# shopetan/mini-kube-scheduler

Hardware: AMD Instinct MI355X
Metric: pod-node evals/sec + pods placed/sec at 5k nodes, 1/2/4/8 MI355X (higher is better)
Workload: dtype u32 (bit-sliced: 32 pod-node pairs per lane-op); 1 GPU; C3 batched: 5000 nodes x 100000 pods per batch per GPU (pod-sharded over 1 GPU); the K batches through msh_schedule_batches_device, 32 per launch, one stream; nodes=5000, parallelism=pod-sharded x1, streams=1, submit=multi (32 batches per launch)

## Files before the change

include/minisched_hip.h:

```cpp
#ifndef MINISCHED_HIP_H
#define MINISCHED_HIP_H

#include <stddef.h>
#include <stdint.h>

#ifdef __cplusplus
extern "C" {
#endif

#define MSH_ABI_VERSION 8

typedef enum msh_err {
  MSH_OK = 0,
  MSH_ERR_INVALID = -1,
  MSH_ERR_NO_DEVICE = -2,
  MSH_ERR_HIP = -3,
  MSH_ERR_STATE = -4,
  MSH_ERR_UNSUPPORTED = -5,
  MSH_ERR_NOMEM = -6
} msh_err;

typedef enum msh_status {
  MSH_PLACED = 0,
  MSH_FIT_ERROR = 1,
  MSH_SCORE_ERROR = 2
} msh_status;

typedef enum msh_plugin_id {
  MSH_PLUGIN_NODE_UNSCHEDULABLE = 1,
  MSH_PLUGIN_NODE_NUMBER = 2,
  MSH_PLUGIN_SCORE_COLUMN0 = 16,
  MSH_PLUGIN_SCORE_COLUMN1 = 17,
  MSH_PLUGIN_SCORE_COLUMN2 = 18,
  MSH_PLUGIN_SCORE_COLUMN3 = 19
} msh_plugin_id;

typedef enum msh_normalize {
  MSH_NORMALIZE_NONE = 0,
  MSH_NORMALIZE_DEFAULT = 1,
  MSH_NORMALIZE_DEFAULT_REVERSE = 2,
  MSH_NORMALIZE_MINMAX = 3
} msh_normalize;

typedef struct msh_ctx msh_ctx;

int msh_abi_version(void);

int msh_device_count(int* out_count);

int msh_host_alloc(size_t bytes, void** out_ptr);
void msh_host_free(void* ptr);

int msh_create(int device, msh_ctx** out_ctx);
void msh_destroy(msh_ctx* ctx);

typedef struct msh_options {
  int32_t struct_size;
  int32_t batch_kernel;
  int32_t pair_planes;
  int32_t pair_noax;
  int32_t pair_slices;
  int32_t seq_waves;
  int32_t seq_split;
  int32_t seq_pod_waves;
  int32_t gen_keys;
  int32_t gen_nnkey;
} msh_options;
int msh_create_ex(int device, const msh_options* opts, msh_ctx** out_ctx);

const char* msh_last_error(const msh_ctx* ctx);

int msh_set_plugins(msh_ctx* ctx, const int32_t* filter_ids, int32_t nf,
                    const int32_t* score_ids, const int64_t* weights, int32_t ns);
int msh_set_plugins_ex(msh_ctx* ctx, const int32_t* filter_ids, int32_t nf,
                       const int32_t* prescore_ids, int32_t npre,
                       const int32_t* score_ids, const int64_t* weights,
                       const int32_t* normalize, int32_t ns);

typedef enum msh_tiebreak { MSH_TIEBREAK_FIRST = 0, MSH_TIEBREAK_RANDOM = 1 } msh_tiebreak;
int msh_set_tiebreak(msh_ctx* ctx, int32_t mode, uint64_t seed, uint64_t counter);
int msh_get_tiebreak(const msh_ctx* ctx, int32_t* out_mode, uint64_t* out_seed, uint64_t* out_counter);

int msh_upload_nodes(msh_ctx* ctx, int32_t n, const uint8_t* unsched, const int8_t* digit);
int msh_num_nodes(const msh_ctx* ctx, int32_t* out_n);

int msh_upload_score_column(msh_ctx* ctx, int32_t plugin_id, int32_t n, const int64_t* scores);

#define MSH_EXPORT_NONE ((int64_t)(-9223372036854775807LL - 1))
int msh_export_results(msh_ctx* ctx, int32_t p, const int8_t* pod_digit, const uint8_t* pod_tol,
                       uint8_t* out_filter, int64_t* out_score, int64_t* out_final);

int msh_patch_nodes(msh_ctx* ctx, int32_t count, const int32_t* idx, const uint8_t* unsched,
                    const int8_t* digit);

int msh_schedule_batch(msh_ctx* ctx, int32_t p, const int8_t* pod_digit, const uint8_t* pod_tol,
                       int32_t* out_idx, int64_t* out_score, int32_t* out_status);

#define MSH_ASYNC_DEPTH 4
int msh_schedule_batch_async(msh_ctx* ctx, int32_t p, const int8_t* pod_digit, const uint8_t* pod_tol,
                             int32_t* out_idx, int64_t* out_score, int32_t* out_status, uint64_t* out_ticket);
int msh_wait(msh_ctx* ctx, uint64_t ticket);

int msh_schedule_batch_device(msh_ctx* ctx, int32_t p, const int8_t* d_pod_digit,
                              const uint8_t* d_pod_tol, int32_t* d_out_idx,
                              int64_t* d_out_score, int32_t* d_out_status, void* stream);

#define MSH_BATCHES_PER_LAUNCH 32
typedef struct msh_batch {
  int32_t p;
  int32_t reserved;
  const int8_t* pod_digit;
  const uint8_t* pod_tol;
  int32_t* out_idx;
  int64_t* out_score;
  int32_t* out_status;
} msh_batch;
int msh_schedule_batches_device(msh_ctx* ctx, int32_t nb, const msh_batch* batches, void* stream);

typedef void (*msh_commit_cb)(void* user, int32_t pod, int32_t node_idx, int64_t score);
// ... 231 lines not shown
```

mini-kube-scheduler_amd/_native.py:

```python
from __future__ import annotations

import ctypes as C
import os
from pathlib import Path

import numpy as np

PKG_DIR = Path(__file__).resolve().parent
LIB_PATH = Path(os.environ.get("MSH_LIBRARY", PKG_DIR / "libminisched_hip.so"))

MSH_OK = 0
MSH_ERR_INVALID = -1
MSH_ERR_NO_DEVICE = -2
MSH_ERR_HIP = -3
MSH_ERR_STATE = -4
MSH_ERR_UNSUPPORTED = -5
MSH_ERR_NOMEM = -6
ERR_NAMES = {
    MSH_ERR_INVALID: "MSH_ERR_INVALID",
    MSH_ERR_NO_DEVICE: "MSH_ERR_NO_DEVICE",
    MSH_ERR_HIP: "MSH_ERR_HIP",
    MSH_ERR_STATE: "MSH_ERR_STATE",
    MSH_ERR_UNSUPPORTED: "MSH_ERR_UNSUPPORTED",
    MSH_ERR_NOMEM: "MSH_ERR_NOMEM",
# ... 45 lines not shown
    "msh_schedule_batches_device", "msh_schedule_sequential",
    "msh_schedule_sequential_device", "msh_node_pod_counts", "msh_reset_node_pod_counts",
    "msh_upload_node_capacity", "msh_patch_node_capacity", "msh_clear_node_capacity", "msh_node_capacity",
    "msh_upload_node_resources", "msh_patch_node_resources", "msh_clear_node_resources", "msh_node_resources",
    "msh_schedule_sequential_fit", "msh_schedule_sequential_fit_device",
    "msh_set_resource_score", "msh_get_resource_score", "msh_seq_fit_max_nodes",
    "msh_upload_node_zones", "msh_clear_node_zones", "msh_node_zones", "msh_set_spread_groups",
    "msh_get_spread_groups", "msh_spread_counts", "msh_patch_spread_counts", "msh_reset_spread_counts",
    "msh_seq_spread_max_nodes", "msh_schedule_sequential_spread", "msh_schedule_sequential_spread_device",
    "msh_seq_spread_scored_max_nodes", "msh_schedule_sequential_spread_scored",
    "msh_schedule_sequential_spread_scored_device",
    "msh_upload_node_class_bits", "msh_patch_node_class_bits", "msh_clear_node_class_bits", "msh_node_class_bits",
    "msh_seq_classes_max_nodes", "msh_schedule_sequential_classes", "msh_schedule_sequential_classes_device",
    "msh_upload_node_class_prefs", "msh_patch_node_class_prefs", "msh_clear_node_class_prefs", "msh_node_class_prefs",
    "msh_set_preference_weights", "msh_preference_weights", "msh_seq_prefs_max_nodes",
    "msh_schedule_sequential_prefs", "msh_schedule_sequential_prefs_device",
    "msh_set_spread_group_modes", "msh_get_spread_group_modes", "msh_set_spread_score_weight", "msh_spread_score_weight",
    "msh_spread_soft_weight", "msh_seq_soft_max_nodes", "msh_schedule_sequential_soft",
    "msh_schedule_sequential_soft_device",
    "msh_set_balanced_score", "msh_balanced_score", "msh_seq_balanced_max_nodes", "msh_schedule_sequential_balanced",
    "msh_schedule_sequential_balanced_device",
    "msh_set_pod_affinity_terms", "msh_get_pod_affinity_terms", "msh_set_pod_profiles", "msh_get_pod_profiles",
    "msh_upload_pod_affinity_state", "msh_patch_pod_affinity_state", "msh_pod_affinity_state",
    "msh_seq_podaffinity_max_nodes", "msh_schedule_sequential_podaffinity", "msh_schedule_sequential_podaffinity_device",
    "msh_shard_keys_len", "msh_shard_keys_device", "msh_decode_keys_device", "msh_keys_slot1_is_any",
    "msh_generic_ext_len", "msh_generic_extents_device", "msh_generic_best_device",
    "msh_generic_candidates_device", "msh_generic_decode_device",
    "msh_comm_unique_id", "msh_comm_init", "msh_comm_info", "msh_schedule_nodeshard_device", "msh_schedule_nodeshard",
    "msh_group_create", "msh_group_destroy", "msh_group_last_error", "msh_group_schedule_batch",
    "msh_timing_begin", "msh_timing_end",
    "msh_pack_nodes", "msh_pack_pods", "msh_toleration_tolerates_unschedulable",
)


class MshError(RuntimeError):
    def __init__(self, code: int, msg: str):
        super().__init__(f"{ERR_NAMES.get(code, code)}: {msg}")
        self.code = code


class Toleration(C.Structure):
    _fields_ = [("key", C.c_char_p), ("op", C.c_char_p), ("value", C.c_char_p), ("effect", C.c_char_p)]


class Batch(C.Structure):
    _fields_ = [("p", C.c_int32), ("reserved", C.c_int32), ("pod_digit", C.c_void_p), ("pod_tol", C.c_void_p),
                ("out_idx", C.c_void_p), ("out_score", C.c_void_p), ("out_status", C.c_void_p)]


class Options(C.Structure):
    _fields_ = [("struct_size", C.c_int32), ("batch_kernel", C.c_int32), ("pair_planes", C.c_int32),
                ("pair_noax", C.c_int32), ("pair_slices", C.c_int32), ("seq_waves", C.c_int32),
                ("seq_split", C.c_int32), ("seq_pod_waves", C.c_int32), ("gen_keys", C.c_int32),
                ("gen_nnkey", C.c_int32)]


OPTION_NAMES = {
    "batch_kernel": {"auto": 0, "pair": 0, "generic": 1},
    "pair_planes": {"auto": 0, "sgpr": 1, "lds": 2},
    "pair_noax": {"auto": 0, "noax": 1, "axlast": 2},
    "pair_slices": {"auto": 0},
    "seq_waves": {"auto": 0},
    "seq_split": {"auto": 0, "serial": 1, "blocks": 2},
    "seq_pod_waves": {"auto": 0},
    "gen_keys": {"auto": 0, "f53": 0, "u64": 1},
    "gen_nnkey": {"auto": 0, "select": 1},
}


def make_options(opts: dict | None) -> "Options | None":
    if not opts:
        return None
    o = Options()
    o.struct_size = C.sizeof(Options)
    for k, v in opts.items():
        if k not in OPTION_NAMES:
            raise ValueError(f"unknown msh_options field {k!r}")
        if isinstance(v, str):
            v = OPTION_NAMES[k][v] if v in OPTION_NAMES[k] else int(v)
        setattr(o, k, int(v))
    return o


COMM_ID_BYTES = 128
GROUP_MAX_SHARDS = 16
BATCHES_PER_LAUNCH = 32
ASYNC_DEPTH = 4

COMMIT_CB = C.CFUNCTYPE(None, C.c_void_p, C.c_int32, C.c_int32, C.c_int64)

_P = C.c_void_p
_I32 = C.c_int32
_I64 = C.c_int64

_SIGS = {
    "msh_abi_version": (C.c_int, []),
    "msh_device_count": (C.c_int, [C.POINTER(C.c_int)]),
    "msh_host_alloc": (C.c_int, [C.c_size_t, C.POINTER(_P)]),
    "msh_host_free": (None, [_P]),
    "msh_create": (C.c_int, [C.c_int, C.POINTER(_P)]),
    "msh_create_ex": (C.c_int, [C.c_int, C.POINTER(Options), C.POINTER(_P)]),
    "msh_destroy": (None, [_P]),
    "msh_last_error": (C.c_char_p, [_P]),
    "msh_set_tiebreak": (C.c_int, [_P, _I32, C.c_uint64, C.c_uint64]),
    "msh_get_tiebreak": (C.c_int, [_P, C.POINTER(_I32), C.POINTER(C.c_uint64), C.POINTER(C.c_uint64)]),
    "msh_set_plugins": (C.c_int, [_P, _P, _I32, _P, _P, _I32]),
    "msh_set_plugins_ex": (C.c_int, [_P, _P, _I32, _P, _I32, _P, _P, _P, _I32]),
    "msh_upload_nodes": (C.c_int, [_P, _I32, _P, _P]),
    "msh_num_nodes": (C.c_int, [_P, C.POINTER(_I32)]),
    "msh_upload_score_column": (C.c_int, [_P, _I32, _I32, _P]),
    "msh_patch_nodes": (C.c_int, [_P, _I32, _P, _P, _P]),
    "msh_export_results": (C.c_int, [_P, _I32, _P, _P, _P, _P, _P]),
    "msh_schedule_batch": (C.c_int, [_P, _I32, _P, _P, _P, _P, _P]),
    "msh_schedule_batch_device": (C.c_int, [_P, _I32, _P, _P, _P, _P, _P, _P]),
    "msh_schedule_batches_device": (C.c_int, [_P, _I32, _P, _P]),
    "msh_schedule_batch_async": (C.c_int, [_P, _I32, _P, _P, _P, _P, _P, C.POINTER(C.c_uint64)]),
    "msh_wait": (C.c_int, [_P, C.c_uint64]),
    "msh_timing_begin": (C.c_int, [_P, _I32]),
    "msh_timing_end": (C.c_int, [_P, C.POINTER(C.c_int32), C.POINTER(C.c_double), C.POINTER(C.c_double)]),
# ... 167 lines not shown
```

mini-kube-scheduler_amd/csrc/msh_capi.cpp:

```cpp
#include <hip/hip_runtime.h>

#include <algorithm>
#include <array>
#include <atomic>
#include <cmath>
#include <condition_variable>
#include <cstdio>
#include <cstdint>
#include <cstdlib>
#include <cstring>
#include <functional>
#include <initializer_list>
#include <iterator>
#include <mutex>
#include <new>
#include <optional>
#include <string>
#include <thread>
#include <vector>

#include "../../include/minisched_hip.h"
#include "msh_ctx.h"
#include "msh_internal.h"
#include "msh_pool.h"
// ... 569 lines not shown
    const CopyJob jobs[2] = {{c->h_stage + L.pd, pod_digit, (size_t)p}, {c->h_stage + L.pt, pod_tol, (size_t)p}};
    par_copy(jobs, 2);
    src_pd = reinterpret_cast<const int8_t*>(c->h_stage + L.pd);
    src_pt = c->h_stage + L.pt;
  }
  io.d_pd = static_cast<int8_t*>(pinned_device_ptr(src_pd));
  io.d_pt = static_cast<uint8_t*>(pinned_device_ptr(src_pt));
  if (!io.d_pd || !io.d_pt) return fail(c, MSH_ERR_HIP, "page-locked pod columns without a device address");
  if (io.staged) {
    io.h_idx = reinterpret_cast<int32_t*>(c->h_stage + L.idx);
    io.h_score = out_score ? reinterpret_cast<int64_t*>(c->h_stage + L.score) : nullptr;
    io.h_status = reinterpret_cast<int32_t*>(c->h_stage + L.status);
    io.o_idx = io.h_idx;
    io.o_score = io.h_score;
    io.o_status = io.h_status;
  } else {
    io.h_idx = out_idx;
    io.h_score = out_score;
    io.h_status = out_status;
    io.o_idx = static_cast<int32_t*>(di);
    io.o_score = static_cast<int64_t*>(ds);
    io.o_status = static_cast<int32_t*>(dt);
  }
  return MSH_OK;
}

int host_io_end(msh_ctx* c, int32_t p, int32_t* out_idx, int64_t* out_score, int32_t* out_status,
                const HostIO& io) {
  MSH_HIP(c, hipStreamSynchronize(c->stream));
  c->async_done = c->async_issued;
  if (io.staged) {
    const CopyJob jobs[3] = {{out_idx, io.h_idx, (size_t)p * sizeof(int32_t)},
                             {out_status, io.h_status, (size_t)p * sizeof(int32_t)},
                             {out_score, io.h_score, (size_t)p * sizeof(int64_t)}};
    par_copy(jobs, out_score ? 3 : 2);
  }
  return MSH_OK;
}

thread_local std::string g_create_err;

bool apply_options(const msh_options& o, msh::DeviceInfo& d, std::string* err) {
  auto in = [&](const char* name, int32_t v, std::initializer_list<int32_t> allowed) {
    for (int32_t a : allowed)
      if (v == a) return true;
    *err = std::string("msh_options.") + name + " = " + std::to_string(v) + ": not one of";
    for (int32_t a : allowed) *err += " " + std::to_string(a);
    return false;
  };
  if (!in("batch_kernel", o.batch_kernel, {0, 1}) || !in("pair_planes", o.pair_planes, {0, 1, 2}) ||
      !in("pair_noax", o.pair_noax, {0, 1, 2}) || !in("pair_slices", o.pair_slices, {0, 1, 2, 4}) ||
      !in("seq_waves", o.seq_waves, {0, 1, 4, 15, 16}) || !in("seq_split", o.seq_split, {0, 1, 2}) ||
      !in("seq_pod_waves", o.seq_pod_waves, {0, 1, 2, 4, 8}) ||
      !in("gen_keys", o.gen_keys, {0, 1}) || !in("gen_nnkey", o.gen_nnkey, {0, 1}))
    return false;
  d.batch_kernel = o.batch_kernel;
  d.pair_planes = o.pair_planes;
  d.pair_noax = o.pair_noax == 0 ? -1 : (o.pair_noax == 1 ? 1 : 0);
  d.bits_slices = o.pair_slices;
  d.seq_waves = o.seq_waves;
  d.seq_split = o.seq_split == 0 ? 2 : (o.seq_split == 1 ? 0 : 1);
  d.seq_pod_waves = o.seq_pod_waves;
  d.gen_f53 = o.gen_keys == 0 ? 1 : 0;
  d.gen_nnkey = o.gen_nnkey == 0 ? 1 : 0;
  return true;
}

}

using namespace msh::capi;

extern "C" {

int msh_abi_version(void) { return MSH_ABI_VERSION; }

int msh_device_count(int* out_count) {
  if (!out_count) return MSH_ERR_INVALID;
  int n = 0;
  hipError_t e = hipGetDeviceCount(&n);
  *out_count = (e == hipSuccess) ? n : 0;
  return MSH_OK;
}

int msh_host_alloc(size_t bytes, void** out_ptr) {
  if (!out_ptr) return MSH_ERR_INVALID;
  *out_ptr = nullptr;
  int n = 0;
  if (hipGetDeviceCount(&n) != hipSuccess || n <= 0) return MSH_ERR_NO_DEVICE;
  const size_t n_bytes = std::max<size_t>(bytes, 1);
  if (hipHostMalloc(out_ptr, n_bytes, hipHostMallocDefault) != hipSuccess) {
    *out_ptr = nullptr;
    return MSH_ERR_NOMEM;
  }
  const uintptr_t a = reinterpret_cast<uintptr_t>(*out_ptr);
  std::lock_guard<std::mutex> g(g_host_mu);
  g_host_allocs.insert(std::upper_bound(g_host_allocs.begin(), g_host_allocs.end(), std::make_pair(a, a)),
                       std::make_pair(a, a + n_bytes));
  return MSH_OK;
}

void msh_host_free(void* ptr) {
  if (!ptr) return;
  {
    const uintptr_t a = reinterpret_cast<uintptr_t>(ptr);
    std::lock_guard<std::mutex> g(g_host_mu);
    auto it = std::lower_bound(g_host_allocs.begin(), g_host_allocs.end(), std::make_pair(a, (uintptr_t)0));
    if (it != g_host_allocs.end() && it->first == a) g_host_allocs.erase(it);
  }
  (void)hipHostFree(ptr);
}

int msh_create(int device, msh_ctx** out_ctx) { return msh_create_ex(device, nullptr, out_ctx); }

int msh_create_ex(int device, const msh_options* opts, msh_ctx** out_ctx) {
  g_create_err.clear();
  if (!out_ctx) return MSH_ERR_INVALID;
  *out_ctx = nullptr;
// ... 1082 lines not shown
```

mini-kube-scheduler_amd/csrc/msh_internal.h:

```cpp
#pragma once

#include <hip/hip_runtime.h>

#include <cstdint>
#include <string>

namespace msh {

constexpr int32_t MAX_NODES = 0xFFFFFE;
constexpr int WAVE = 64;
constexpr int32_t GKEY_MAX = 0x7FFFFFFF;
constexpr uint32_t NOFIT = 0x80000000u;

struct PluginParams {
  int32_t has_nu_filter;
  int32_t has_nn_score;
  int32_t nn_prescore;
  int32_t mode;
  int64_t weight;
};

inline bool needs_kx(const PluginParams& pp) {
  return pp.has_nn_score && pp.nn_prescore && (pp.mode == 2 || pp.mode == 3);
}

struct DeviceInfo {
  int cus = 256;
  int bits_slices = 0;
  int seq_waves = 0;
  int batch_kernel = 0;
  int pair_planes = 0;
  int pair_noax = -1;
  int seq_split = 2;
  int seq_pod_waves = 0;
  int gen_f53 = 1;
  int gen_nnkey = 1;
};

constexpr uint32_t CODE_NONE_NODE = 15u;
constexpr uint32_t CODE_NONE_POD = 14u;

constexpr int PLANE_GW = 8;
constexpr int PLANE_N = 6;
constexpr int PLANE_X = 4, PLANE_V = 5;
constexpr int GROUP_NODES = PLANE_GW * 32;
constexpr int GROUP_DWORDS = PLANE_GW * PLANE_N;
constexpr int32_t NODE_PAD = 1024;

hipError_t launch_node_prep(const uint8_t* d_unsched, const int8_t* d_digit, int32_t n, int32_t n_pad,
                            int32_t has_nu, uint32_t* d_planes, hipStream_t s);
constexpr int PATCH_INLINE = 64;
struct TableCopyArgs {
  const uint8_t* src_unsched;
  const int8_t* src_digit;
  const uint32_t* src_planes;
  uint8_t* dst_unsched;
  int8_t* dst_digit;
  uint32_t* dst_planes;
  int32_t n, n_words, has_nu, count;
  unsigned long long inl[PATCH_INLINE];
};
hipError_t launch_table_copy(const TableCopyArgs& a, hipStream_t s);
hipError_t launch_patch_scatter(const unsigned long long* d_entries, int32_t count, uint8_t* d_unsched,
                                int8_t* d_digit, hipStream_t s);

constexpr int64_t EXPORT_NONE = INT64_MIN;
hipError_t launch_export(const uint8_t* d_unsched, const int8_t* d_digit, int32_t n,
                         const int8_t* d_pod_digit, const uint8_t* d_pod_tol, int32_t p,
                         const PluginParams& pp, uint8_t* d_filter, int64_t* d_raw, int64_t* d_fin,
                         hipStream_t s);

struct BatchDesc {
  const int8_t* pod_digit;
  const uint8_t* pod_tol;
  int32_t* out_idx;
  int64_t* out_score;
  int32_t* out_status;
  int32_t n_pods;
  int32_t reserved;
};
constexpr int MULTI_MAX = 32;

struct PairCommon {
  const uint32_t* planes;
  int32_t n_groups;
  int32_t g_full;
  int32_t gps;
  int32_t noax;
  int32_t nb;
  PluginParams pp;
  int64_t node_base;
  int32_t* keys;
  int32_t* counts;
  int64_t count_stride;
};
template <int NB>
struct PairArgsN : PairCommon {
  BatchDesc d[NB];
};
using PairArgs = PairArgsN<MULTI_MAX>;
hipError_t launch_pairs(PairArgs& a, bool shard, const DeviceInfo& dev, hipStream_t s);

struct PickArgs {
  const uint32_t* planes;
  int32_t n_groups;
  int32_t nb;
  PluginParams pp;
  uint64_t seed;
  BatchDesc d[MULTI_MAX];
  uint64_t draw_base[MULTI_MAX];
};
constexpr int TIEBREAK_LDS_MAX_GROUPS = 416;
hipError_t launch_pair_pick(const PickArgs& a, hipStream_t s);

hipError_t launch_decode_keys(const int8_t* pod_digit, int32_t p, const int32_t* keys, PluginParams pp,
                              int32_t* out_idx, int64_t* out_score, int32_t* out_status, hipStream_t s);

constexpr int GROUP_MAX = 16;
struct GroupPtrs {
  const int32_t* keys[GROUP_MAX];
  const int64_t* v[GROUP_MAX];
  const int32_t* idx[GROUP_MAX];
  int32_t n;
};
hipError_t launch_group_keys_decode(const GroupPtrs& g, const int8_t* pod_digit, int32_t p, PluginParams pp,
                                    int32_t* out_idx, int64_t* out_score, int32_t* out_status, hipStream_t s);
hipError_t launch_group_max_i64(const GroupPtrs& g, int64_t len, int64_t* out, hipStream_t s);
hipError_t launch_group_best_merge(const GroupPtrs& g, int32_t p, int64_t* out_total, int32_t* out_idx,
                                   hipStream_t s);

constexpr int GEN_MAX_SCORE = 5;
constexpr int GEN_COLS = 4;
struct GenericArgs {
// ... 171 lines not shown
```

mini-kube-scheduler_amd/csrc/msh_pair.hip:

```cpp
#include "msh_device.h"

namespace msh {

template <int NPL>
__device__ __forceinline__ void sload_group(u32x8* pl, const uint32_t* src) {
#pragma unroll
  for (int k = 0; k < NPL; ++k)
    asm volatile("s_load_dwordx8 %0, %1, %2" : "=s"(pl[k]) : "s"(src), "n"(k * PLANE_GW * 4));
  if constexpr (NPL == 5)
    asm volatile("s_waitcnt lgkmcnt(0)" : "+s"(pl[0]), "+s"(pl[1]), "+s"(pl[2]), "+s"(pl[3]), "+s"(pl[4]));
  else
    asm volatile("s_waitcnt lgkmcnt(0)" : "+s"(pl[0]), "+s"(pl[1]), "+s"(pl[2]), "+s"(pl[3]), "+s"(pl[4]),
                 "+s"(pl[5]));
}

__device__ __forceinline__ void sload_xv(u32x8 (&pl)[PLANE_N], const uint32_t* grp) {
  asm volatile("s_load_dwordx8 %0, %2, %3\n\ts_load_dwordx8 %1, %2, %4\n\ts_waitcnt lgkmcnt(0)"
               : "=&s"(pl[PLANE_X]), "=&s"(pl[PLANE_V])
               : "s"(grp), "n"(PLANE_X * PLANE_GW * 4), "n"(PLANE_V * PLANE_GW * 4));
}

template <int NPL, bool LDSP>
__device__ __forceinline__ void get_group(u32x8* pl, const uint32_t* planes, const uint4* s_tab, int32_t g) {
  if constexpr (LDSP) {
// ... 305 lines not shown
      uint32_t u = TY == 0 ? bop3_or_xor(pl[PLANE_X][ww], pl[0][ww], P0) : (pl[0][ww] ^ P0);
      u = bop3_or_xor(u, pl[1][ww], P1);
      u = bop3_or_xor(u, pl[2][ww], P2);
      t[h] = bop3_or_xor(u, pl[3][ww], P3);
    }
    am = bop3_and3(am, t[0], t[1]);
#pragma unroll
    for (int h = 0; h < 2; ++h) {
      const int ww = w + h;
      if constexpr (KX) {
        if constexpr (TY == 0) ax = PAD ? (ax | bop3_andn_and(t[h], pl[PLANE_X][ww], pl[PLANE_V][ww]))
                                       : bop3_or_andn(ax, t[h], pl[PLANE_X][ww]);
        else ax = PAD ? (ax | (t[h] & pl[PLANE_V][ww])) : (ax | t[h]);
      }
    }
  }
}

template <bool KX, int TY>
__device__ __forceinline__ void pair_group_hy(const uint32_t (&pl)[PLANE_N][PLANE_GW], const u32x8& X,
                                              const u32x8& D3, uint32_t P0, uint32_t P1, uint32_t P2, uint32_t P3,
                                              uint32_t nT, uint32_t& am, uint32_t& ax) {
#pragma unroll
  for (int w = 0; w < PLANE_GW; w += 2) {
    uint32_t t[2], xi[2];
#pragma unroll
    for (int h = 0; h < 2; ++h) {
      const int ww = w + h;
      uint32_t u;
      if constexpr (TY == 0) {
        u = bop3_or_xor(X[ww], pl[0][ww], P0);
      } else if constexpr (TY == 1) {
        u = pl[0][ww] ^ P0;
      } else {
        xi[h] = __builtin_amdgcn_bitop3_b32(X[ww], nT, nT, 0xc0);
        u = bop3_or_xor(xi[h], pl[0][ww], P0);
      }
      u = bop3_or_xor(u, pl[1][ww], P1);
      u = bop3_or_xor(u, pl[2][ww], P2);
      t[h] = bop3_or_xor(u, D3[ww], P3);
    }
    am = bop3_and3(am, t[0], t[1]);
    if constexpr (KX) {
#pragma unroll
      for (int h = 0; h < 2; ++h) {
        if constexpr (TY == 0) ax = bop3_or_andn(ax, t[h], X[w + h]);
        else if constexpr (TY == 1) ax |= t[h];
        else ax = bop3_or_andn(ax, t[h], xi[h]);
      }
    }
  }
}

template <int KIND>
__device__ __forceinline__ uint32_t group_first_lds(const uint4* __restrict__ s_tab, uint32_t g, uint32_t P0,
                                                    uint32_t P1, uint32_t P2, uint32_t P3, uint32_t nT) {
  const uint4* q = s_tab + g * (GROUP_DWORDS / 4);
#pragma unroll 1
  for (int hh = 0; hh < 2; ++hh) {
    uint32_t pl[PLANE_N][4];
#pragma unroll
    for (int k = 0; k < PLANE_N; ++k) {
      const uint4 v = q[2 * k + hh];
      pl[k][0] = v.x; pl[k][1] = v.y; pl[k][2] = v.z; pl[k][3] = v.w;
    }
    uint32_t t[4];
#pragma unroll
    for (int c = 0; c < 4; ++c) {
      const uint32_t fe = ~(pl[PLANE_X][c] & nT) & pl[PLANE_V][c];
      const uint32_t dm = (pl[0][c] ^ P0) | (pl[1][c] ^ P1) | (pl[2][c] ^ P2) | (pl[3][c] ^ P3);
      const uint32_t h = KIND == 1 ? (dm & fe) : (~dm & fe);
      t[c] = lowbit(h) | (uint32_t)(32 * c);
    }
    const uint32_t m = umin(umin(t[0], t[1]), umin(t[2], t[3]));
    if (m < 128u) return g * GROUP_NODES + (uint32_t)(hh * 128) + m;
  }
  return NOFIT;
}

template <bool KX>
__device__ __forceinline__ void group_firsts_lds(const uint4* __restrict__ s_tab, uint32_t g, uint32_t P0,
                                                 uint32_t P1, uint32_t P2, uint32_t P3, uint32_t nT, bool digit,
                                                 uint32_t& rm, uint32_t& rx) {
  const uint4* q = s_tab + g * (GROUP_DWORDS / 4);
  uint32_t bm = 0xFFFFFFFFu, bx = 0xFFFFFFFFu;
  if constexpr (!KX) {
    constexpr int PLX = 4;
    static_assert(PLANE_X == PLX, "X follows the four code planes");
    auto half = [&](auto hc) -> uint32_t {
      constexpr int hh = decltype(hc)::value;
      uint32_t pl[PLX + 1][4];
#pragma unroll
      for (int k = 0; k <= PLX; ++k) {
        const uint4 v = q[2 * k + hh];
        pl[k][0] = v.x; pl[k][1] = v.y; pl[k][2] = v.z; pl[k][3] = v.w;
      }
      uint32_t t[4];
#pragma unroll
      for (int c = 0; c < 4; ++c) {
        uint32_t u = __builtin_amdgcn_bitop3_b32(pl[PLX][c], nT, nT, 0xc0);
        u = bop3_or_xor(u, pl[0][c], P0);
        u = bop3_or_xor(u, pl[1][c], P1);
        u = bop3_or_xor(u, pl[2][c], P2);
        u = __builtin_amdgcn_bitop3_b32(u, pl[3][c], P3, 0x09);
        t[c] = lowbit(u);
        if (c + 4 * hh != 0) t[c] |= (uint32_t)(32 * (c + 4 * hh));
      }
      return umin(umin(t[0], t[1]), umin(t[2], t[3]));
    };
    bm = half(std::integral_constant<int, 0>{});
    if (__ballot(digit && bm == 0xFFFFFFFFu) != 0) bm = umin(bm, half(std::integral_constant<int, 1>{}));
    rm = bm < GROUP_NODES ? g * GROUP_NODES + bm : NOFIT;
    return;
  }
#pragma unroll 1
  for (int hh = 0; hh < 2; ++hh) {
    uint32_t pl[PLANE_N][4];
#pragma unroll
    for (int k = 0; k < PLANE_N; ++k) {
      const uint4 v = q[2 * k + hh];
      pl[k][0] = v.x; pl[k][1] = v.y; pl[k][2] = v.z; pl[k][3] = v.w;
    }
#pragma unroll
    for (int c = 0; c < 4; ++c) {
      const uint32_t fe = ~(pl[PLANE_X][c] & nT) & pl[PLANE_V][c];
      const uint32_t dm = (pl[0][c] ^ P0) | (pl[1][c] ^ P1) | (pl[2][c] ^ P2) | (pl[3][c] ^ P3);
      const uint32_t off = (uint32_t)(32 * (c + 4 * hh));
      bm = umin(bm, lowbit(~dm & fe) | off);
      if constexpr (KX) bx = umin(bx, lowbit(dm & fe) | off);
    }
    if (hh == 0 && __ballot((digit && bm == 0xFFFFFFFFu) || (KX && bx == 0xFFFFFFFFu)) == 0) break;
  }
  rm = bm < GROUP_NODES ? g * GROUP_NODES + bm : NOFIT;
  if constexpr (KX) rx = bx < GROUP_NODES ? g * GROUP_NODES + bx : NOFIT;
}

template <bool SHARD, bool KX, int W>
__global__ __launch_bounds__(W * WAVE) void pair_lds_kernel(PairArgs a) {
  constexpr bool CMP = KX && W == PL_WAVES;
  constexpr int HY = KX ? 2 : 1;
  extern __shared__ uint4 s_tab[];
  constexpr int NSL = W * PL_BPW;
  __shared__ uint32_t s_cnt[CMP ? NSL : 1];
  __shared__ uint32_t s_pod[CMP ? NSL * WAVE : 1];
  const BatchDesc& d = a.d[blockIdx.y];
  const int32_t np = d.n_pods;
  const int32_t wg0 = (int32_t)blockIdx.x * NSL * WAVE;
  if (wg0 >= np) return;
  {
    const uint4* __restrict__ src = reinterpret_cast<const uint4*>(a.planes);
    const int32_t nq = a.n_groups * (GROUP_DWORDS / 4);
    for (int32_t i = threadIdx.x; i < nq; i += W * WAVE) s_tab[i] = src[i];
  }
  const int lane = threadIdx.x & (WAVE - 1);
  const int wv = __builtin_amdgcn_readfirstlane((int)(threadIdx.x >> 6));
  const int32_t n_groups = a.n_groups, g_full = a.g_full;
  uint32_t pk[PL_BPW];
#pragma unroll
  for (int b = 0; b < PL_BPW; ++b) {
    const int32_t pos0 = (wv * PL_BPW + b) * WAVE + lane;
    const int32_t j = wg0 + pos0;
    uint32_t c = CODE_NONE_POD, t = 0u;
    if (j < np) {
      const int dq = d.pod_digit[j];
      c = (dq >= 0 && dq <= 9) ? (uint32_t)dq : CODE_NONE_POD;
      t = d.pod_tol[j] ? 1u : 0u;
    }
    pk[b] = ((uint32_t)pos0 << 8) | (t << 4) | c;
  }
  if constexpr (CMP) {
    uint64_t mn[PL_BPW];
#pragma unroll
    for (int b = 0; b < PL_BPW; ++b) {
      mn[b] = __ballot(((pk[b] >> 4) & 1u) == 0u);
      if (lane == 0) s_cnt[wv * PL_BPW + b] = (uint32_t)__builtin_popcountll(mn[b]);
    }
    __syncthreads();
    uint32_t tot = 0, pre[PL_BPW];
#pragma unroll
    for (int k = 0; k < NSL; ++k) {
      const uint32_t c = s_cnt[k];
#pragma unroll
      for (int b = 0; b < PL_BPW; ++b)
        if (k == wv * PL_BPW + b) pre[b] = tot;
      tot += c;
    }
#pragma unroll
    for (int b = 0; b < PL_BPW; ++b) {
      const uint32_t sl = (uint32_t)(wv * PL_BPW + b);
      const bool nt = ((pk[b] >> 4) & 1u) == 0u;
      const uint32_t below = nt ? __builtin_amdgcn_mbcnt_hi((uint32_t)(mn[b] >> 32), __builtin_amdgcn_mbcnt_lo((uint32_t)mn[b], 0u))
                                : __builtin_amdgcn_mbcnt_hi((uint32_t)(~mn[b] >> 32), __builtin_amdgcn_mbcnt_lo((uint32_t)~mn[b], 0u));
      const uint32_t pos = nt ? pre[b] + below : tot + (sl * WAVE - pre[b]) + below;
      s_pod[pos] = pk[b];
    }
    __syncthreads();
#pragma unroll
    for (int b = 0; b < PL_BPW; ++b) pk[b] = s_pod[(wv * PL_BPW + b) * WAVE + lane];
  } else {
    __syncthreads();
  }
  uint32_t P0[PL_BPW], P1[PL_BPW], P2[PL_BPW], P3[PL_BPW], nT[PL_BPW], code[PL_BPW];
  int32_t jj[PL_BPW];
  int ty[PL_BPW];
  bool any_act = false;
#pragma unroll
  for (int b = 0; b < PL_BPW; ++b) {
    const uint32_t c = pk[b] & 15u, t = (pk[b] >> 4) & 1u;
    jj[b] = wg0 + (int32_t)(pk[b] >> 8);
    code[b] = c;
    P0[b] = 0u - (c & 1u);
    P1[b] = 0u - ((c >> 1) & 1u);
    P2[b] = 0u - ((c >> 2) & 1u);
    P3[b] = 0u - (c >> 3);
    nT[b] = t ? 0u : 0xFFFFFFFFu;
    const uint64_t tm = __ballot(t != 0u);
    ty[b] = CMP ? (tm == 0 ? 0 : (~tm == 0 ? 1 : 2)) : 2;
    any_act = any_act || __ballot(jj[b] < np) != 0;
  }
  if (!any_act) return;
  uint32_t fm[PL_BPW], fx[PL_BPW], amw[PL_BPW];
#pragma unroll
  for (int b = 0; b < PL_BPW; ++b) {
    fm[b] = fx[b] = NO_GROUP;
    amw[b] = 0xFFFFFFFFu;
  }
  uint32_t fn = NO_GROUP, ft = NO_GROUP;
  uint32_t rm[PL_BPW], rx[PL_BPW];
  auto group0 = [&]() {
#pragma unroll
    for (int b = 0; b < PL_BPW; ++b) group_firsts_lds<KX>(s_tab, 0u, P0[b], P1[b], P2[b], P3[b], nT[b], code[b] != CODE_NONE_POD, rm[b], rx[b]);
  };
  auto scan = [&](auto noax) {
    constexpr bool NOAX = decltype(noax)::value;
    constexpr bool KXS = KX && !NOAX;
    for (int32_t g = n_groups - 1; g > 0; g -= 2) {
      uint32_t ams[PL_BPW], ax[PL_BPW];
      uint32_t(&am)[PL_BPW] = *(KX ? &ams : &amw);
#pragma unroll
      for (int b = 0; b < PL_BPW; ++b) {
        if constexpr (KX) am[b] = 0xFFFFFFFFu;
        ax[b] = 0u;
      }
      const int32_t g2 = g - 1 > 0 ? g - 1 : g;
      u32x8 spp[2][2];
      if constexpr (HY == 2) {
        asm volatile("s_load_dwordx8 %0, %4, %6\n\ts_load_dwordx8 %1, %4, %7\n\t"
                     "s_load_dwordx8 %2, %5, %6\n\ts_load_dwordx8 %3, %5, %7\n\ts_waitcnt lgkmcnt(0)"
                     : "=&s"(spp[0][0]), "=&s"(spp[0][1]), "=&s"(spp[1][0]), "=&s"(spp[1][1])
                     : "s"(a.planes + (size_t)g * GROUP_DWORDS), "s"(a.planes + (size_t)g2 * GROUP_DWORDS),
                       "n"(PLANE_X * PLANE_GW * 4), "n"(3 * PLANE_GW * 4));
      }
#pragma unroll
      for (int h = 0; h < 2; ++h) {
        const int32_t gg = h == 0 ? g : g - 1;
        if (h == 1 && gg <= 0) break;
        uint32_t pl[PLANE_N][PLANE_GW];
        if (!KX || gg < g_full) {
          u32x8 sp[2];
          if constexpr (HY == 2) {
            sp[0] = spp[h][0];
            sp[1] = spp[h][1];
          } else {
            asm volatile("s_load_dwordx8 %0, %2, %3\n\ts_load_dwordx8 %1, %2, %4\n\ts_waitcnt lgkmcnt(0)"
                         : "=&s"(sp[0]), "=&s"(sp[1])
                         : "s"(a.planes + (size_t)gg * GROUP_DWORDS), "n"(PLANE_X * PLANE_GW * 4), "n"(3 * PLANE_GW * 4));
          }
          lds_group<3>(pl, s_tab, gg);
#pragma unroll
          for (int b = 0; b < PL_BPW; ++b) {
            if (ty[b] == 0) pair_group_hy<KXS, 0>(pl, sp[0], sp[1], P0[b], P1[b], P2[b], P3[b], nT[b], am[b], ax[b]);
            else if (ty[b] == 1) pair_group_hy<KXS, 1>(pl, sp[0], sp[1], P0[b], P1[b], P2[b], P3[b], nT[b], am[b], ax[b]);
            else pair_group_hy<KXS, 2>(pl, sp[0], sp[1], P0[b], P1[b], P2[b], P3[b], nT[b], am[b], ax[b]);
          }
          if constexpr (!KX) {
            if (gg < g_full) {
              const uint32_t axg = sp[0][0] & sp[0][1] & sp[0][2] & sp[0][3] & sp[0][4] & sp[0][5] & sp[0][6] & sp[0][7];
              fn = axg != 0xFFFFFFFFu ? (uint32_t)gg : fn;
              ft = (uint32_t)gg;
            } else {
              u32x8 xv[PLANE_N];
              bool sn, st;
              sload_xv(xv, a.planes + (size_t)gg * GROUP_DWORDS);
              group_feasible_s<true>(xv, sn, st);
              fn = sn ? (uint32_t)gg : fn;
              ft = st ? (uint32_t)gg : ft;
            }
          }
        } else {
          lds_group<PLANE_N>(pl, s_tab, gg);
#pragma unroll
          for (int b = 0; b < PL_BPW; ++b) {
            if (ty[b] == 0) pair_group_ty<true, KXS, 0>(pl, P0[b], P1[b], P2[b], P3[b], am[b], ax[b]);
            else if (ty[b] == 1) pair_group_ty<true, KXS, 1>(pl, P0[b], P1[b], P2[b], P3[b], am[b], ax[b]);
            else pair_group_v<true, KXS>(pl, P0[b], P1[b], P2[b], P3[b], nT[b], am[b], ax[b]);
          }
        }
      }
      if constexpr (KX) {
#pragma unroll
        for (int b = 0; b < PL_BPW; ++b) {
          fm[b] = am[b] != 0xFFFFFFFFu ? (uint32_t)g2 : fm[b];
          if constexpr (KXS) fx[b] = ax[b] != 0u ? (uint32_t)g2 : fx[b];
        }
      }
    }
  };
  if constexpr (!KX) {
    scan(std::false_type{});
    group0();
    u32x8 xv[PLANE_N];
    sload_xv(xv, a.planes);
    uint32_t an = group_first_feasible_s<true>(xv, 0u);
    uint32_t at = group_first_feasible_s<false>(xv, 0u);
    if (an == NOFIT && fn != NO_GROUP) {
      sload_xv(xv, a.planes + (size_t)fn * GROUP_DWORDS);
      an = group_first_feasible_s<true>(xv, fn);
    }
    if (at == NOFIT && ft != NO_GROUP) {
      sload_xv(xv, a.planes + (size_t)ft * GROUP_DWORDS);
      at = group_first_feasible_s<false>(xv, ft);
    }
#pragma unroll
    for (int b = 0; b < PL_BPW; ++b) rx[b] = nT[b] ? an : at;
  } else if (a.noax) {
    group0();
    bool xdone = true;
#pragma unroll
    for (int b = 0; b < PL_BPW; ++b) xdone = xdone && __ballot(rx[b] == NOFIT) == 0;
    if (xdone) scan(std::true_type{});
    else scan(std::false_type{});
  } else {
    scan(std::false_type{});
    group0();
  }
#pragma unroll
  for (int b = 0; b < PL_BPW; ++b) {
    const int32_t j = jj[b];
    if (__ballot(j < np) == 0) continue;
    if constexpr (!KX) {
      bool pend = rm[b] == NOFIT && amw[b] != 0xFFFFFFFFu;
      for (int32_t g = 1; g < n_groups && __ballot(pend) != 0; ++g) {
        if (pend) {
          rm[b] = group_first_lds<0>(s_tab, (uint32_t)g, P0[b], P1[b], P2[b], P3[b], nT[b]);
          pend = rm[b] == NOFIT;
        }
      }
    } else if (rm[b] == NOFIT && fm[b] != NO_GROUP) {
      rm[b] = group_first_lds<0>(s_tab, fm[b], P0[b], P1[b], P2[b], P3[b], nT[b]);
      if (rm[b] == NOFIT) rm[b] = group_first_lds<0>(s_tab, fm[b] + 1, P0[b], P1[b], P2[b], P3[b], nT[b]);
    }
    if constexpr (KX) {
      if (rx[b] == NOFIT && fx[b] != NO_GROUP) {
        rx[b] = group_first_lds<1>(s_tab, fx[b], P0[b], P1[b], P2[b], P3[b], nT[b]);
        if (rx[b] == NOFIT) rx[b] = group_first_lds<1>(s_tab, fx[b] + 1, P0[b], P1[b], P2[b], P3[b], nT[b]);
      }
    }
    if (j < np) {
      if constexpr (SHARD) {
        a.keys[j] = rm[b] != NOFIT ? shard_key(a.node_base, rm[b]) : 0;
        a.keys[(size_t)np + j] = rx[b] != NOFIT ? shard_key(a.node_base, rx[b]) : 0;
      } else {
        const uint32_t ra = umin(rm[b], rx[b]);
        int32_t oi, ost;
        int64_t osc;
        decode_pod(rm[b] != NOFIT ? (int64_t)rm[b] : -1, (KX && rx[b] != NOFIT) ? (int64_t)rx[b] : -1,
                   ra != NOFIT ? (int64_t)ra : -1, code[b] != CODE_NONE_POD, a.pp, &oi, &osc, &ost);
        d.out_idx[j] = oi;
        if (d.out_score) d.out_score[j] = osc;
        d.out_status[j] = ost;
      }
    }
  }
}

namespace {
int pair_slices(int64_t waves, int32_t n_groups, const DeviceInfo& dev) {
  if (dev.bits_slices > 0) return dev.bits_slices;
  const int64_t want = (int64_t)dev.cus * 4 * 4;
  int sl = 1;
  while (sl < PAIR_WAVES && waves * sl < want && n_groups >= 4 * sl) sl *= 2;
  return sl;
}

template <int S, bool SHARD, bool KX, bool LDSP>
hipError_t launch_pair_l(PairArgs& a, int32_t bx, hipStream_t s) {
  a.gps = (a.n_groups + S - 1) / S;
  const dim3 grid((unsigned)bx, (unsigned)a.nb), blk(PAIR_WAVES * WAVE);
  const unsigned lds = LDSP ? (unsigned)(a.n_groups * GROUP_DWORDS * sizeof(uint32_t)) : 0u;
  if (a.nb == 1) {
    PairArgsN<1> b;
    static_cast<PairCommon&>(b) = a;
    b.d[0] = a.d[0];
    if (a.counts) {
      if constexpr (SHARD) return hipErrorInvalidValue;
      else MSH_TIMED_LAUNCH((pair_kernel<S, false, KX, true, 1, LDSP>), grid, blk, lds, s, b);
    } else {
      MSH_TIMED_LAUNCH((pair_kernel<S, SHARD, KX, false, 1, LDSP>), grid, blk, lds, s, b);
    }
    return hipGetLastError();
  }
  if constexpr (SHARD) return hipErrorInvalidValue;
  else MSH_TIMED_LAUNCH((pair_kernel<S, false, KX, false, MULTI_MAX, LDSP>), grid, blk, lds, s, a);
  return hipGetLastError();
}

constexpr int PAIR_SLICE_LDS_GROUPS = 128;
template <int S, bool SHARD, bool KX>
hipError_t launch_pair_s(PairArgs& a, int32_t bx, const DeviceInfo& dev, hipStream_t s) {
  if (dev.pair_planes != 1 && a.n_groups <= PAIR_SLICE_LDS_GROUPS) return launch_pair_l<S, SHARD, KX, true>(a, bx, s);
  return launch_pair_l<S, SHARD, KX, false>(a, bx, s);
}

template <bool SHARD, bool KX>
hipError_t launch_pair_t(PairArgs& a, const DeviceInfo& dev, hipStream_t s) {
  int32_t maxp = 0;
  int64_t waves = 0;
  for (int b = 0; b < a.nb; ++b) {
    maxp = std::max(maxp, a.d[b].n_pods);
    waves += (a.d[b].n_pods + WAVE - 1) / WAVE;
  }
  if (maxp == 0) return hipSuccess;
  const bool fits = a.n_groups <= PAIR_LDS_MAX_GROUPS;
  const bool big = !fits && a.n_groups <= PAIR_LDS_BIG_GROUPS;
  const int64_t min_waves = (int64_t)dev.cus * (big ? 2 * PL_WAVES_BIG : 64);
  const bool lds = !a.counts && (fits || big) && (dev.pair_planes == 2 ||
                                     (dev.pair_planes == 0 && waves >= min_waves && dev.bits_slices == 0));
  if (lds) {
    const int w = big ? PL_WAVES_BIG : PL_WAVES;
    const int32_t blocks = (maxp + WAVE - 1) / WAVE;
    const int32_t bx = (blocks + w * PL_BPW - 1) / (w * PL_BPW);
    const size_t bytes = (size_t)a.n_groups * GROUP_DWORDS * sizeof(uint32_t);
    const dim3 grid((unsigned)bx, (unsigned)a.nb), blk(w * WAVE);
    a.noax = dev.pair_noax >= 0 ? dev.pair_noax : (KX ? 1 : 0);
    using PairKernel = void (*)(PairArgs);
    const PairKernel k = big ? pair_lds_kernel<SHARD, KX, PL_WAVES_BIG> : pair_lds_kernel<SHARD, KX, PL_WAVES>;
    if (bytes > 64 * 1024) {
      hipError_t e = hipFuncSetAttribute(reinterpret_cast<const void*>(k), hipFuncAttributeMaxDynamicSharedMemorySize, (int)bytes);
      if (e != hipSuccess) return e;
    }
    MSH_TIMED_LAUNCH(k, grid, blk, (unsigned)bytes, s, a);
    return hipGetLastError();
  }
  const int S = pair_slices(waves, a.n_groups, dev);
  const int32_t blocks = (maxp + WAVE - 1) / WAVE;
  auto bx = [&](int sl) { return (blocks * sl + PAIR_WAVES - 1) / PAIR_WAVES; };
  switch (S) {
    case 1: return launch_pair_s<1, SHARD, KX>(a, bx(1), dev, s);
    case 2: return launch_pair_s<2, SHARD, KX>(a, bx(2), dev, s);
    default: return launch_pair_s<4, SHARD, KX>(a, bx(4), dev, s);
  }
}
}

hipError_t launch_pairs(PairArgs& a, bool shard, const DeviceInfo& dev, hipStream_t s) {
  if (a.nb <= 0 || a.nb > MULTI_MAX || (shard && a.nb != 1) || (a.counts && (shard || a.nb != 1)))
    return hipErrorInvalidValue;
  if (needs_kx(a.pp)) return shard ? launch_pair_t<true, true>(a, dev, s) : launch_pair_t<false, true>(a, dev, s);
  return shard ? launch_pair_t<true, false>(a, dev, s) : launch_pair_t<false, false>(a, dev, s);
}

}
```

Before: 210900 billion pod-node evals/s.

## Sort pods by class in LDS kernel and fold planes for pure waves

In the non-KX LDS pair kernel, pods are compacted inside each block by whether bits 0x18 of their code are clear. Waves whose pods are all of this class and untainted then use a cheaper folded-plane check that ORs two plane vectors once per group and skips the taint path. The goal is fewer ALU ops per group in the hot scan for the common pod class. The cost is an extra block-level shuffle through LDS with two syncthreads, plus more scan template instances and larger code size.

```diff
diff --git a/include/minisched_hip.h b/include/minisched_hip.h
--- a/include/minisched_hip.h
+++ b/include/minisched_hip.h
@@ -65,6 +65,7 @@
   int32_t seq_pod_waves;
   int32_t gen_keys;
   int32_t gen_nnkey;
+  int32_t pair_fold;
 } msh_options;
 int msh_create_ex(int device, const msh_options* opts, msh_ctx** out_ctx);
 
diff --git a/mini-kube-scheduler_amd/_native.py b/mini-kube-scheduler_amd/_native.py
--- a/mini-kube-scheduler_amd/_native.py
+++ b/mini-kube-scheduler_amd/_native.py
@@ -121,7 +121,7 @@
     _fields_ = [("struct_size", C.c_int32), ("batch_kernel", C.c_int32), ("pair_planes", C.c_int32),
                 ("pair_noax", C.c_int32), ("pair_slices", C.c_int32), ("seq_waves", C.c_int32),
                 ("seq_split", C.c_int32), ("seq_pod_waves", C.c_int32), ("gen_keys", C.c_int32),
-                ("gen_nnkey", C.c_int32)]
+                ("gen_nnkey", C.c_int32), ("pair_fold", C.c_int32)]
 
 
 OPTION_NAMES = {
@@ -134,6 +134,7 @@
     "seq_pod_waves": {"auto": 0},
     "gen_keys": {"auto": 0, "f53": 0, "u64": 1},
     "gen_nnkey": {"auto": 0, "select": 1},
+    "pair_fold": {"auto": 0, "on": 0, "off": 1},
 }
 
 
diff --git a/mini-kube-scheduler_amd/csrc/msh_capi.cpp b/mini-kube-scheduler_amd/csrc/msh_capi.cpp
--- a/mini-kube-scheduler_amd/csrc/msh_capi.cpp
+++ b/mini-kube-scheduler_amd/csrc/msh_capi.cpp
@@ -645,7 +645,8 @@
       !in("pair_noax", o.pair_noax, {0, 1, 2}) || !in("pair_slices", o.pair_slices, {0, 1, 2, 4}) ||
       !in("seq_waves", o.seq_waves, {0, 1, 4, 15, 16}) || !in("seq_split", o.seq_split, {0, 1, 2}) ||
       !in("seq_pod_waves", o.seq_pod_waves, {0, 1, 2, 4, 8}) ||
-      !in("gen_keys", o.gen_keys, {0, 1}) || !in("gen_nnkey", o.gen_nnkey, {0, 1}))
+      !in("gen_keys", o.gen_keys, {0, 1}) || !in("gen_nnkey", o.gen_nnkey, {0, 1}) ||
+      !in("pair_fold", o.pair_fold, {0, 1}))
     return false;
   d.batch_kernel = o.batch_kernel;
   d.pair_planes = o.pair_planes;
@@ -656,6 +657,7 @@
   d.seq_pod_waves = o.seq_pod_waves;
   d.gen_f53 = o.gen_keys == 0 ? 1 : 0;
   d.gen_nnkey = o.gen_nnkey == 0 ? 1 : 0;
+  d.pair_fold = o.pair_fold == 0 ? 1 : 0;
   return true;
 }
 
diff --git a/mini-kube-scheduler_amd/csrc/msh_internal.h b/mini-kube-scheduler_amd/csrc/msh_internal.h
--- a/mini-kube-scheduler_amd/csrc/msh_internal.h
+++ b/mini-kube-scheduler_amd/csrc/msh_internal.h
@@ -31,6 +31,7 @@
   int batch_kernel = 0;
   int pair_planes = 0;
   int pair_noax = -1;
+  int pair_fold = 1;
   int seq_split = 2;
   int seq_pod_waves = 0;
   int gen_f53 = 1;
@@ -79,6 +80,7 @@
   int32_t n_pods;
   int32_t reserved;
 };
+constexpr int32_t PAIR_FLAG_FOLD = 2;
 constexpr int MULTI_MAX = 32;
 
 struct PairCommon {
diff --git a/mini-kube-scheduler_amd/csrc/msh_pair.hip b/mini-kube-scheduler_amd/csrc/msh_pair.hip
--- a/mini-kube-scheduler_amd/csrc/msh_pair.hip
+++ b/mini-kube-scheduler_amd/csrc/msh_pair.hip
@@ -381,6 +381,25 @@
   }
 }
 
+typedef uint64_t u64x4 __attribute__((ext_vector_type(4)));
+__device__ __forceinline__ u32x8 fold_planes(const u32x8& X, const u32x8& D3) {
+  return __builtin_bit_cast(u32x8, __builtin_bit_cast(u64x4, X) | __builtin_bit_cast(u64x4, D3));
+}
+__device__ __forceinline__ void pair_group_fold(const uint32_t (&pl)[PLANE_N][PLANE_GW], const u32x8& S, uint32_t P0,
+                                                uint32_t P1, uint32_t P2, uint32_t& am) {
+#pragma unroll
+  for (int w = 0; w < PLANE_GW; w += 2) {
+    uint32_t t[2];
+#pragma unroll
+    for (int h = 0; h < 2; ++h) {
+      uint32_t u = bop3_or_xor(S[w + h], pl[0][w + h], P0);
+      u = bop3_or_xor(u, pl[1][w + h], P1);
+      t[h] = bop3_or_xor(u, pl[2][w + h], P2);
+    }
+    am = bop3_and3(am, t[0], t[1]);
+  }
+}
+
 template <int KIND>
 __device__ __forceinline__ uint32_t group_first_lds(const uint4* __restrict__ s_tab, uint32_t g, uint32_t P0,
                                                     uint32_t P1, uint32_t P2, uint32_t P3, uint32_t nT) {
@@ -467,11 +486,13 @@
 template <bool SHARD, bool KX, int W>
 __global__ __launch_bounds__(W * WAVE) void pair_lds_kernel(PairArgs a) {
   constexpr bool CMP = KX && W == PL_WAVES;
+  constexpr bool FOLD = !KX && W == PL_WAVES;
   constexpr int HY = KX ? 2 : 1;
   extern __shared__ uint4 s_tab[];
   constexpr int NSL = W * PL_BPW;
-  __shared__ uint32_t s_cnt[CMP ? NSL : 1];
-  __shared__ uint32_t s_pod[CMP ? NSL * WAVE : 1];
+  __shared__ uint32_t s_cnt[(CMP || FOLD) ? NSL : 1];
+  __shared__ uint32_t s_pod[(CMP || FOLD) ? NSL * WAVE : 1];
+  const bool fold = FOLD && (a.noax & PAIR_FLAG_FOLD) != 0;
   const BatchDesc& d = a.d[blockIdx.y];
   const int32_t np = d.n_pods;
   const int32_t wg0 = (int32_t)blockIdx.x * NSL * WAVE;
@@ -526,12 +547,45 @@
     __syncthreads();
 #pragma unroll
     for (int b = 0; b < PL_BPW; ++b) pk[b] = s_pod[(wv * PL_BPW + b) * WAVE + lane];
+  } else if constexpr (FOLD) {
+    if (fold) {
+      uint64_t m0[PL_BPW];
+#pragma unroll
+      for (int b = 0; b < PL_BPW; ++b) {
+        m0[b] = __ballot((pk[b] & 0x18u) == 0u);
+        if (lane == 0) s_cnt[wv * PL_BPW + b] = (uint32_t)__builtin_popcountll(m0[b]);
+      }
+      __syncthreads();
+      uint32_t tot = 0, pre[PL_BPW];
+#pragma unroll
+      for (int k = 0; k < NSL; ++k) {
+        const uint32_t c = (uint32_t)__builtin_amdgcn_readfirstlane((int)s_cnt[k]);
+#pragma unroll
+        for (int b = 0; b < PL_BPW; ++b)
+          if (k == wv * PL_BPW + b) pre[b] = tot;
+        tot += c;
+      }
+#pragma unroll
+      for (int b = 0; b < PL_BPW; ++b) {
+        const uint32_t sl = (uint32_t)(wv * PL_BPW + b);
+        const bool c0 = (pk[b] & 0x18u) == 0u;
+        const uint64_t mk = c0 ? m0[b] : ~m0[b];
+        const uint32_t below = __builtin_amdgcn_mbcnt_hi((uint32_t)(mk >> 32), __builtin_amdgcn_mbcnt_lo((uint32_t)mk, 0u));
+        s_pod[(c0 ? pre[b] : tot + (sl * WAVE - pre[b])) + below] = pk[b];
+      }
+      __syncthreads();
+#pragma unroll
+      for (int b = 0; b < PL_BPW; ++b) pk[b] = s_pod[(wv * PL_BPW + b) * WAVE + lane];
+    } else {
+      __syncthreads();
+    }
   } else {
     __syncthreads();
   }
   uint32_t P0[PL_BPW], P1[PL_BPW], P2[PL_BPW], P3[PL_BPW], nT[PL_BPW], code[PL_BPW];
   int32_t jj[PL_BPW];
   int ty[PL_BPW];
+  bool pure[PL_BPW];
   bool any_act = false;
 #pragma unroll
   for (int b = 0; b < PL_BPW; ++b) {
@@ -545,6 +599,8 @@
     nT[b] = t ? 0u : 0xFFFFFFFFu;
     const uint64_t tm = __ballot(t != 0u);
     ty[b] = CMP ? (tm == 0 ? 0 : (~tm == 0 ? 1 : 2)) : 2;
+    const uint64_t pm = FOLD ? __ballot((c >> 3) != 0u) : 0;
+    pure[b] = fold && tm == 0 && pm == 0;
     any_act = any_act || __ballot(jj[b] < np) != 0;
   }
   if (!any_act) return;
@@ -560,8 +616,9 @@
 #pragma unroll
     for (int b = 0; b < PL_BPW; ++b) group_firsts_lds<KX>(s_tab, 0u, P0[b], P1[b], P2[b], P3[b], nT[b], code[b] != CODE_NONE_POD, rm[b], rx[b]);
   };
-  auto scan = [&](auto noax) {
+  auto scan = [&](auto noax, auto fsel) {
     constexpr bool NOAX = decltype(noax)::value;
+    constexpr int FSEL = decltype(fsel)::value;
     constexpr bool KXS = KX && !NOAX;
     for (int32_t g = n_groups - 1; g > 0; g -= 2) {
       uint32_t ams[PL_BPW], ax[PL_BPW];
@@ -596,6 +653,14 @@
                          : "s"(a.planes + (size_t)gg * GROUP_DWORDS), "n"(PLANE_X * PLANE_GW * 4), "n"(3 * PLANE_GW * 4));
           }
           lds_group<3>(pl, s_tab, gg);
+          if constexpr (FSEL != 0) {
+            const u32x8 S = fold_planes(sp[0], sp[1]);
+#pragma unroll
+            for (int b = 0; b < PL_BPW; ++b) {
+              if ((FSEL >> b) & 1) pair_group_fold(pl, S, P0[b], P1[b], P2[b], am[b]);
+              else pair_group_hy<false, 2>(pl, sp[0], sp[1], P0[b], P1[b], P2[b], P3[b], nT[b], am[b], ax[b]);
+            }
+          } else
 #pragma unroll
           for (int b = 0; b < PL_BPW; ++b) {
             if (ty[b] == 0) pair_group_hy<KXS, 0>(pl, sp[0], sp[1], P0[b], P1[b], P2[b], P3[b], nT[b], am[b], ax[b]);
@@ -636,7 +701,16 @@
     }
   };
   if constexpr (!KX) {
-    scan(std::false_type{});
+    using F0 = std::integral_constant<int, 0>;
+    if constexpr (FOLD) {
+      static_assert(PL_BPW == 2, "one scan instance per subset of the wave's blocks");
+      if (pure[0] && pure[1]) scan(std::false_type{}, std::integral_constant<int, 3>{});
+      else if (pure[0]) scan(std::false_type{}, std::integral_constant<int, 1>{});
+      else if (pure[1]) scan(std::false_type{}, std::integral_constant<int, 2>{});
+      else scan(std::false_type{}, F0{});
+    } else {
+      scan(std::false_type{}, F0{});
+    }
     group0();
     u32x8 xv[PLANE_N];
     sload_xv(xv, a.planes);
@@ -657,10 +731,10 @@
     bool xdone = true;
 #pragma unroll
     for (int b = 0; b < PL_BPW; ++b) xdone = xdone && __ballot(rx[b] == NOFIT) == 0;
-    if (xdone) scan(std::true_type{});
-    else scan(std::false_type{});
+    if (xdone) scan(std::true_type{}, std::integral_constant<int, 0>{});
+    else scan(std::false_type{}, std::integral_constant<int, 0>{});
   } else {
-    scan(std::false_type{});
+    scan(std::false_type{}, std::integral_constant<int, 0>{});
     group0();
   }
 #pragma unroll
@@ -762,6 +836,7 @@
     const size_t bytes = (size_t)a.n_groups * GROUP_DWORDS * sizeof(uint32_t);
     const dim3 grid((unsigned)bx, (unsigned)a.nb), blk(w * WAVE);
     a.noax = dev.pair_noax >= 0 ? dev.pair_noax : (KX ? 1 : 0);
+    if (!KX && dev.pair_fold) a.noax |= PAIR_FLAG_FOLD;
     using PairKernel = void (*)(PairArgs);
     const PairKernel k = big ? pair_lds_kernel<SHARD, KX, PL_WAVES_BIG> : pair_lds_kernel<SHARD, KX, PL_WAVES>;
     if (bytes > 64 * 1024) {
```

Measured after the change: 230300 billion pod-node evals/s (median of 6 runs). +9.2%, better.
